# microsoft/ORBIT-Dataset

Measured on AMD Instinct MI355X. Metric: query frames/sec per task (224×224, 5-way ProtoNet) + frame accuracy vs ref, higher is better.
Workload: dtype f32

## Files before the change

include/orbit_hip.h:

```cpp
#ifndef ORBIT_HIP_H
#define ORBIT_HIP_H

#include <stddef.h>
#include <stdint.h>

#ifdef __cplusplus
extern "C" {
#endif

typedef struct orbit_extractor orbit_extractor_t;
typedef struct orbit_filmgen orbit_filmgen_t;
typedef void* orbit_stream_t;

#define ORBIT_OK 0
#define ORBIT_ERR_ARG (-1)
#define ORBIT_ERR_HIP (-2)
#define ORBIT_ERR_STATE (-3)
#define ORBIT_ERR_NOMEM (-4)

#define ORBIT_ACT_NONE 0
#define ORBIT_ACT_RELU 1
#define ORBIT_ACT_SILU 2
#define ORBIT_ACT_ELU 3

// ... 37 lines not shown

int orbit_extractor_load(orbit_extractor_t* fe, const char* key, const float* data, size_t numel);
int orbit_extractor_load_async(orbit_extractor_t* fe, const char* key, const float* device_data, size_t numel,
                               orbit_stream_t stream);
int orbit_extractor_load_all_async(orbit_extractor_t* fe, const float* const* device_ptrs, int n, orbit_stream_t stream);
int orbit_extractor_finalize(orbit_extractor_t* fe, orbit_stream_t stream);

int orbit_extractor_output_size(const orbit_extractor_t* fe);
int orbit_extractor_film_slots(const orbit_extractor_t* fe);
int orbit_extractor_film_slot_channels(const orbit_extractor_t* fe, int slot);
const char* orbit_extractor_film_slot_name(const orbit_extractor_t* fe, int slot);
int orbit_extractor_film_size(const orbit_extractor_t* fe);

size_t orbit_extractor_workspace_bytes(const orbit_extractor_t* fe, int B);
double orbit_extractor_macs_per_frame(const orbit_extractor_t* fe);

int orbit_extractor_forward(orbit_extractor_t* fe, const float* frames, int B,
                            const float* film_gamma, const float* film_beta,
                            float* feats, void* workspace, size_t workspace_bytes, orbit_stream_t stream);

int orbit_filmgen_create(int n_gen, int z_dim, int hidden, const int* out_size, const int* kind,
                         const int* dst_offset, orbit_filmgen_t** out);
void orbit_filmgen_destroy(orbit_filmgen_t* g);
int orbit_filmgen_load(orbit_filmgen_t* g, int gen, const char* tensor, const float* data, size_t numel);
int orbit_filmgen_load_all_async(orbit_filmgen_t* g, const float* const* device_ptrs, int n, orbit_stream_t stream);
int orbit_filmgen_forward(orbit_filmgen_t* g, const float* z, float* film_gamma, float* film_beta,
                          float* l2, orbit_stream_t stream);

int orbit_op_conv2d(const float* x, int x_nchw, const float* w, float* y,
                    const float* scale, const float* shift, const float* residual, const float* gate,
                    int B, int H, int W, int Cin, int Cout, int KH, int KW, int stride,
                    int pad_top, int pad_left, int Ho, int Wo, int act, int pool2,
                    orbit_stream_t stream);
int orbit_op_dwconv2d(const float* x, const float* w, float* y, const float* scale, const float* shift,
                      int B, int H, int W, int C, int K, int stride, int pad_top, int pad_left,
                      int Ho, int Wo, int act, orbit_stream_t stream);
int orbit_op_conv2d_train(const float* x, int x_nchw, const float* w, float* y, const float* gate, int B, int H, int W,
                          int Cin, int Cout, int KH, int KW, int stride, int pad_top, int pad_left, int Ho, int Wo,
                          float* stats, int* stat_blocks, orbit_stream_t stream);
int orbit_op_dwconv2d_train(const float* x, const float* w, float* y, const float* in_scale, const float* in_shift,
                            int in_act, int B, int H, int W, int C, int K, int stride, int pad_top, int pad_left, int Ho,
                            int Wo, float* stats, orbit_stream_t stream);
int orbit_op_maxpool2d(const float* x, float* y, int B, int H, int W, int C, int K, int stride, int pad,
                       int Ho, int Wo, orbit_stream_t stream);
int orbit_op_avgpool(const float* x, float* y, int B, int HW, int C, orbit_stream_t stream);
int orbit_op_se_gate(const float* pooled, const float* w1, const float* b1, const float* w2,
                     const float* b2, float* gate, int B, int C, int R, orbit_stream_t stream);

int orbit_op_mbconv_front_partials(int H, int W, int Cin, int mid, int K, int stride);
int orbit_op_mbconv_front(const float* x, const float* w1, const float* scale1, const float* shift1,
                          const float* wdw, const float* scale2, const float* shift2, float* y, float* pool_partial,
                          int B, int H, int W, int Cin, int mid, int K, int stride, int pad_top, int pad_left,
                          int Ho, int Wo, orbit_stream_t stream);
int orbit_op_stem_dw_front_partials(int H, int W, int mid);
int orbit_op_stem_dw_front(const float* frames, const float* w_stem, const float* scale1, const float* shift1,
                           const float* wdw, const float* scale2, const float* shift2, float* y, float* pool_partial,
                           int B, int FH, int FW, int spad_top, int spad_left, int H, int W, int mid, int pad_top,
                           int pad_left, int Ho, int Wo, orbit_stream_t stream);

int orbit_dense_rows(const float* x, int R, int in, const float* W, const float* b, int out, int act,
                     const float* residual, float* y, orbit_stream_t stream);
int orbit_spd_inverse(const float* A, float* Ainv, int n, int batch, orbit_stream_t stream);
size_t orbit_mahalanobis_workspace_bytes(int N, int M, int D, int C);
int orbit_mahalanobis_configure(const float* features, const int64_t* labels, const int64_t* class_ids, int N, int D,
                                int C, float* means, float* task_mean, float* precisions, float* task_precision,
                                void* workspace, size_t workspace_bytes, orbit_stream_t stream);
// ... 115 lines not shown
```

orbit-dataset_amd/_lib.py:

```python
import ctypes
import os
from ctypes import c_char_p, c_double, c_float, c_int, c_size_t, c_void_p, POINTER

_HERE = os.path.dirname(os.path.abspath(__file__))
LIB_PATH = os.path.join(_HERE, "lib", "liborbit_hip.so")

_lib = None

P = c_void_p
_SIGNATURES = {
    "orbit_version": (c_int, []),
    "orbit_last_error": (c_char_p, []),
    "orbit_device_count": (c_int, []),
    "orbit_set_option": (c_int, [c_char_p, c_int]),
    "orbit_get_option": (c_int, [c_char_p]),
    "orbit_label_set": (c_int, [P, c_int, P, c_int, P, P]),
    "orbit_proto_configure": (c_int, [P, P, P, c_int, c_int, c_int, c_int, c_int, P, P, P]),
    "orbit_proto_finalize": (c_int, [P, P, c_int, c_int, c_int, c_int, P, P, P]),
    "orbit_proto_predict": (c_int, [P, P, P, c_int, c_int, c_int, c_int, c_int, c_float, c_int, P, P, P]),
    "orbit_mean_pool": (c_int, [P, c_int, c_int, c_int, P, P]),
    "orbit_set_mean": (c_int, [P, c_int, c_int, P, P]),
    "orbit_history_mean_pool": (c_int, [P, c_int, c_int, c_int, P, P]),
    "orbit_extractor_create": (c_int, [c_char_p, c_int, c_int, POINTER(c_void_p)]),
    "orbit_extractor_create_ex": (c_int, [c_char_p, c_int, c_int, c_int, POINTER(c_void_p)]),
    "orbit_extractor_destroy": (None, [P]),
    "orbit_extractor_num_params": (c_int, [P]),
    "orbit_extractor_param_name": (c_char_p, [P, c_int]),
    "orbit_extractor_param_numel": (c_size_t, [P, c_int]),
    "orbit_extractor_load": (c_int, [P, c_char_p, P, c_size_t]),
    "orbit_extractor_load_async": (c_int, [P, c_char_p, P, c_size_t, P]),
    "orbit_extractor_load_all_async": (c_int, [P, P, c_int, P]),
    "orbit_extractor_finalize": (c_int, [P, P]),
    "orbit_extractor_output_size": (c_int, [P]),
    "orbit_extractor_film_slots": (c_int, [P]),
    "orbit_extractor_film_slot_channels": (c_int, [P, c_int]),
    "orbit_extractor_film_slot_name": (c_char_p, [P, c_int]),
    "orbit_extractor_film_size": (c_int, [P]),
    "orbit_extractor_workspace_bytes": (c_size_t, [P, c_int]),
    "orbit_extractor_macs_per_frame": (c_double, [P]),
    "orbit_extractor_forward": (c_int, [P, P, c_int, P, P, P, P, c_size_t, P]),
    "orbit_filmgen_create": (c_int, [c_int, c_int, c_int, POINTER(c_int), POINTER(c_int), POINTER(c_int),
                                     POINTER(c_void_p)]),
    "orbit_filmgen_destroy": (None, [P]),
    "orbit_filmgen_load": (c_int, [P, c_int, c_char_p, P, c_size_t]),
    "orbit_filmgen_load_all_async": (c_int, [P, P, c_int, P]),
    "orbit_filmgen_forward": (c_int, [P, P, P, P, P, P]),
    "orbit_op_conv2d": (c_int, [P, c_int, P, P, P, P, P, P] + [c_int] * 14 + [P]),
    "orbit_op_dwconv2d": (c_int, [P, P, P, P, P] + [c_int] * 11 + [P]),
    "orbit_op_conv2d_train": (c_int, [P, c_int, P, P, P] + [c_int] * 12 + [P, POINTER(c_int), P]),
    "orbit_op_dwconv2d_train": (c_int, [P, P, P, P, P] + [c_int] * 11 + [P, P]),
    "orbit_op_maxpool2d": (c_int, [P, P] + [c_int] * 9 + [P]),
    "orbit_op_avgpool": (c_int, [P, P, c_int, c_int, c_int, P]),
    "orbit_op_se_gate": (c_int, [P, P, P, P, P, P, c_int, c_int, c_int, P]),
    "orbit_op_mbconv_front": (c_int, [P] * 9 + [c_int] * 11 + [P]),
    "orbit_op_mbconv_front_partials": (c_int, [c_int] * 6),
    "orbit_op_stem_dw_front_partials": (c_int, [c_int] * 3),
    "orbit_op_stem_dw_front": (c_int, [P] * 9 + [c_int] * 12 + [P]),
    "orbit_dense_rows": (c_int, [P, c_int, c_int, P, P, c_int, c_int, P, P, P]),
    "orbit_spd_inverse": (c_int, [P, P, c_int, c_int, P]),
    "orbit_mahalanobis_workspace_bytes": (c_size_t, [c_int, c_int, c_int, c_int]),
    "orbit_mahalanobis_configure": (c_int, [P, P, P, c_int, c_int, c_int, P, P, P, P, P, c_size_t, P]),
    "orbit_mahalanobis_predict": (c_int, [P, P, P, c_int, c_int, c_int, c_float, P, P, c_size_t, P]),
    "orbit_mahalanobis_predict_backward": (c_int, [P, P, P, P, c_int, c_int, c_int, c_float, P, P, c_size_t, P]),
    "orbit_extractor_supports_training": (c_int, [P]),
    "orbit_extractor_tape_bytes": (c_size_t, [P, c_int]),
    "orbit_extractor_backward_workspace_bytes": (c_size_t, [P, c_int]),
    "orbit_extractor_grad_floats": (c_size_t, [P]),
    "orbit_extractor_param_offset": (c_size_t, [P, c_int]),
    "orbit_extractor_bn_stat_floats": (c_size_t, [P]),
    "orbit_extractor_export_bn_stats": (c_int, [P, P, P]),
    "orbit_extractor_train_forward": (c_int, [P, P, c_int, P, P, c_int, c_float, P, P, c_size_t, P]),
    "orbit_extractor_train_forward_ex": (c_int, [P, P, c_int, P, P, c_int, c_float, P, P, c_size_t, c_int, P]),
    "orbit_extractor_apply_deferred_bn_stats": (c_int, [P, P, c_size_t, c_int, c_float, P]),
    "orbit_extractor_backward": (c_int, [P, P, c_int, P, P, c_int, P, P, c_size_t, P, c_int, P, P, P, c_size_t, P]),
    "orbit_filmgen_grad_floats": (c_size_t, [P]),
    "orbit_filmgen_param_offset": (c_size_t, [P, c_int, c_char_p]),
    "orbit_filmgen_backward": (c_int, [P, P, P, P, P, P, P, P]),
    "orbit_proto_predict_backward": (c_int, [P, P, P, c_int, c_int, c_int, c_int, c_float, c_int, P, P]),
    "orbit_linear_head_backward": (c_int, [P, P, c_int, c_int, c_int, c_float, P, P, P]),
    "orbit_cross_entropy_forward": (c_int, [P, P, c_int, c_int, c_int, P, P, P, P]),
    "orbit_cross_entropy_backward": (c_int, [P, P, P, c_int, c_int, c_int, P, P]),
# ... 160 lines not shown
```

orbit-dataset_amd/build.py:

```python
import hashlib
import os
import subprocess
import sys
from concurrent.futures import ThreadPoolExecutor

HERE = os.path.dirname(os.path.abspath(__file__))
CSRC = os.path.join(HERE, "csrc")
LIBDIR = os.path.join(HERE, "lib")
OBJDIR = os.path.join(HERE, "build")
LIB = os.path.join(LIBDIR, "liborbit_hip.so")
INCLUDE = os.path.join(os.path.dirname(HERE), "include")

SOURCES = ["head.hip", "heads_extra.hip", "loss.hip", "conv_igemm.hip", "pw_rgemm.hip", "conv_bf3.hip", "ops.hip", "film.hip", "ingest.hip", "mbconv_rows.hip", "stem.hip", "extractor.hip", "train_ops.hip", "train_mbconv.hip", "conv_wgrad.hip", "extractor_train.hip",
           "comm.hip"]
HIPCC = os.environ.get("HIPCC", "/opt/rocm/bin/hipcc")
FLAGS = ["--offload-arch=gfx950", "-O3", "-std=c++17", "-fPIC", "-Wall", "-Wno-unused-function",
         "-I", INCLUDE, "-I", "/opt/rocm/include"]


def _runtime_libdir():
    if os.environ.get("ORBIT_SYSTEM_ROCM") == "1":
        return "/opt/rocm/lib"
    try:
        import torch
        d = os.path.join(os.path.dirname(torch.__file__), "lib")
        if os.path.exists(os.path.join(d, "libamdhip64.so")):
            return d
    except Exception:
        pass
    return "/opt/rocm/lib"


RTLIB = _runtime_libdir()
LINK = ["-shared", "-fPIC", "--offload-arch=gfx950", "-no-hip-rt", "-L" + RTLIB, "-lamdhip64", "-lrccl",
        "-Wl,-rpath," + RTLIB, "-Wl,--no-undefined"]


def _digest(paths):
    root = os.path.dirname(HERE)
    h = hashlib.sha256()
    for p in sorted(paths):
        with open(p, "rb") as f:
            h.update(os.path.relpath(p, root).encode())
            h.update(f.read())
    h.update(" ".join(x.replace(root, "<repo>") for x in FLAGS + LINK).encode())
    return h.hexdigest()
# ... 48 lines not shown
```

orbit-dataset_amd/csrc/common.h:

```cpp
#pragma once
#include <hip/hip_runtime.h>
#include <cstdarg>
#include <cstdio>
#include <cstdint>
#include <cstring>
#include "../../include/orbit_hip.h"

namespace orbit {

char* err_buf();
int set_err(int code, const char* fmt, ...);
int get_option(const char* name);
int option_epoch();

#define ORBIT_HIP_CHECK(expr)                                                                  \
    do {                                                                                       \
        hipError_t _e = (expr);                                                                \
        if (_e != hipSuccess)                                                                  \
            return ::orbit::set_err(ORBIT_ERR_HIP, "%s failed: %s (%s:%d)", #expr,             \
                                    hipGetErrorString(_e), __FILE__, __LINE__);                \
    } while (0)

#define ORBIT_LAUNCH_CHECK()                                                                   \
    do {                                                                                       \
// ... 36 lines not shown
    const float* gate;
    int B, H, W, Cin, Cout, KH, KW, stride, pad_t, pad_l, Ho, Wo;
    int act;
    int pool2;
    int x_nchw;
    float prof_flop_scale = 1.f;
    float* splitk_ws = nullptr;
    float* stats = nullptr;
    int* stats_blocks = nullptr;
    bool stats_only = false;
    float* y_raw = nullptr;
};
inline size_t conv_stats_floats(size_t M, int Cout) { return ((M + 31) / 32) * 2 * (size_t)Cout; }
int conv_splitk(const ConvDesc& d);
size_t conv_splitk_floats(const ConvDesc& d);

struct ConvPackGeom {
    int cin_pad;
    int kt;
    int cout_pad;
};
ConvPackGeom conv_pack_geom(int Cin, int Cout, int KH, int KW, int x_nchw);
size_t conv_packed_floats(int Cin, int Cout, int KH, int KW, int x_nchw);
int conv_pack_weights(const float* w_oihw, float* w_packed, int Cin, int Cout, int KH, int KW,
                      int x_nchw, hipStream_t s);
int launch_conv(const ConvDesc& d, hipStream_t s);
size_t conv_frag_floats(int Cin, int Cout, int KH, int KW, int x_nchw);
int conv_frag_pack_weights(const float* w_oihw, float* w_frag, int Cin, int Cout, hipStream_t s);
bool pw_rgemm_supported(const ConvDesc& d);
bool conv_bf3_supported(const ConvDesc& d);
int launch_conv_bf3(const ConvDesc& d, hipStream_t s);
bool pw_rgemm_preferred(const ConvDesc& d);
int launch_pw_rgemm(const ConvDesc& d, hipStream_t s);
bool conv_prof_enabled();
int prof_start(const char* name, double flops, double bytes, hipStream_t s, double silu = 0.0);
void prof_stop(int idx, hipStream_t s);

struct DwBnBwd {
    const float* y = nullptr;
    const float* mean = nullptr;
    const float* invstd = nullptr;
    const float* scale = nullptr;
    const float* shift = nullptr;
    int act = 0;
    float* partial = nullptr;
    int* nblk = nullptr;
    float* wgrad_partial = nullptr;
    int* wgrad_rows = nullptr;
};
int dwconv_se_chunks(int Ho);
int launch_dwconv_se(const float* x, const float* w_khwc, float* y, const float* scale, const float* shift,
                     float* pool_partial, int B, int H, int W, int C, int K, int stride, int pad_t, int pad_l, int Ho,
                     int Wo, int act, hipStream_t s, int stats = 0, const float* in_scale = nullptr,
                     const float* in_shift = nullptr, int in_act = 0, const DwBnBwd* bnb = nullptr);
int launch_se_gate2(const float* partial, int chunks, int HW, const float* w1, const float* b1, const float* w2t,
                    const float* b2, float* gate, int B, int C, int R, hipStream_t s, float* pooled_out = nullptr);
int launch_transpose(const float* in, float* out, int rows, int cols, hipStream_t s);
bool stem_direct_supported(int Cin, int Cout, int K, int stride, int W, int act);
int launch_stem_direct(const float* frames, const float* w_oihw, const float* scale, const float* shift, float* y, int B,
                       int H, int W, int pad_t, int pad_l, int Ho, int Wo, hipStream_t s);
bool mbconv_rows_supported(int H, int W, int Cin, int mid, int K, int stride);
int mbconv_rows_tiles(int H, int W, int Cin, int mid, int K, int stride);
int launch_mbconv_rows(const float* x, const float* w1, const float* sc1, const float* sh1, const float* wdw,
                       const float* sc2, const float* sh2, float* y, float* pool, int B, int H, int W, int Cin, int mid,
                       int K, int stride, int pad_t, int pad_l, int Ho, int Wo, hipStream_t s, int plan_tiles = 0,
                       bool raw_stats = false);
// ... 114 lines not shown
```

orbit-dataset_amd/csrc/extractor.hip:

```cpp
#include <chrono>
#include <cstdlib>

#include "extractor.h"

using namespace orbit;

static int conv_out(int H, int K, int stride, int pad) { return (H + 2 * pad - K) / stride + 1; }
static void same_pad(int H, int K, int stride, int& Ho, int& pad_before) {
    Ho = (H + stride - 1) / stride;
    const int total = std::max((Ho - 1) * stride + K - H, 0);
    pad_before = total / 2;
}

static int build_resnet18(orbit_extractor* fe, int H, int W) {
    fe->out_size = 512;
    int h = conv_out(H, 7, 2, 3), w = conv_out(W, 7, 2, 3);
    int bn = fe->add_bn("bn1", 64, 1e-5f, true);
    fe->add_conv("conv1.weight", bn, -1, 0, -1, H, W, 3, 64, 7, 2, 3, 3, h, w, ORBIT_ACT_RELU, 0, 1, 0);
    {
        Op o;
        o.kind = OP_MAXPOOL, o.in = 0, o.out = 1, o.H = h, o.W = w, o.Cin = 64, o.Cout = 64;
        o.pool_k = 3, o.stride = 2, o.pool_pad = 1;
        o.Ho = conv_out(h, 3, 2, 1), o.Wo = conv_out(w, 3, 2, 1);
        h = o.Ho, w = o.Wo;
// ... 472 lines not shown
    }
    hit->stamp = ++fe->graph_clock;
    if (hit->exec == nullptr) {
        hipGraph_t graph = nullptr;
        if (fe->cap_stream == nullptr)
            ORBIT_HIP_CHECK(hipStreamCreateWithFlags(&fe->cap_stream, hipStreamNonBlocking));
        if (hipStreamBeginCapture(fe->cap_stream, hipStreamCaptureModeThreadLocal) != hipSuccess) {
            (void)hipGetLastError();
            return run_plan(fe, frames, B, film_gamma, film_beta, feats, workspace, s);
        }
        const int rc = run_plan(fe, frames, B, film_gamma, film_beta, feats, workspace, fe->cap_stream);
        const hipError_t ce = hipStreamEndCapture(fe->cap_stream, &graph);
        if (rc != ORBIT_OK) {
            if (graph) (void)hipGraphDestroy(graph);
            return rc;
        }
        if (ce != hipSuccess || graph == nullptr) {
            (void)hipGetLastError();
            return run_plan(fe, frames, B, film_gamma, film_beta, feats, workspace, s);
        }
        hipGraphExec_t exec = nullptr;
        const hipError_t ie = hipGraphInstantiate(&exec, graph, nullptr, nullptr, 0);
        (void)hipGraphDestroy(graph);
        if (ie != hipSuccess || exec == nullptr) {
            (void)hipGetLastError();
            return run_plan(fe, frames, B, film_gamma, film_beta, feats, workspace, s);
        }
        hit->exec = exec;
    }
    ORBIT_HIP_CHECK(hipGraphLaunch(hit->exec, s));
    return ORBIT_OK;
}

static int run_plan(orbit_extractor_t* fe, const float* frames, int B, const float* film_gamma, const float* film_beta,
                    float* feats, void* workspace, hipStream_t s) {
    const WsLayout L = ws_layout(fe, B);
    char* ws = static_cast<char*>(workspace);
    auto buf = [&](int id) -> float* {
        if (id == -1) return const_cast<float*>(frames);
        if (id == 100) return feats;
        if (id == 101) return reinterpret_cast<float*>(ws + L.pooled);
        if (id == 102) return reinterpret_cast<float*>(ws + L.gate);
        return reinterpret_cast<float*>(ws + L.buf[id]);
    };
    const float* scale = fe->d_fold;
    const float* shift = fe->d_fold + fe->fold_floats;
    if (film_gamma && fe->film_size > 0) {
        float* fs = reinterpret_cast<float*>(ws + L.fold);
        dim3 grid((unsigned)fe->bns.size(), 2);
        const int rec = prof_start("bn_fold_film", 0.0, 4.0 * 6.0 * fe->fold_floats, s);
        bn_fold_all_kernel<<<grid, 256, 0, s>>>(fe->d_bn, fe->d_pool, film_gamma, film_beta, fs, fs + fe->fold_floats);
        prof_stop(rec, s);
        ORBIT_LAUNCH_CHECK();
        scale = fs, shift = fs + fe->fold_floats;
    }
    for (size_t oi = 0; oi < fe->ops.size(); ++oi) {
        const Op& o = fe->ops[oi];
        int rc = ORBIT_OK;
        switch (o.kind) {
            case OP_CONV: {
                if (o.x_nchw && !o.pool2 && o.res < 0 && o.bn >= 0 &&
                    stem_direct_supported(o.Cin, o.Cout, o.KH, o.stride, o.W, o.act) && o.KH == o.KW) {
                    rc = launch_stem_direct(buf(o.in), fe->d_pool + fe->params[o.weight].off, scale + fe->bns[o.bn].fold_off,
                                            shift + fe->bns[o.bn].fold_off, buf(o.out), B, o.H, o.W, o.pad_t, o.pad_l, o.Ho,
                                            o.Wo, s);
                    break;
                }
                ConvDesc d;
                d.x = buf(o.in), d.w_packed = fe->d_packed + o.packed_off, d.y = buf(o.out);
                d.w_frag = o.frag_off != SIZE_MAX ? fe->d_packed + o.frag_off : nullptr;
                d.scale = o.bn >= 0 ? scale + fe->bns[o.bn].fold_off : nullptr;
                d.shift = o.bn >= 0 ? shift + fe->bns[o.bn].fold_off : nullptr;
                d.residual = o.res >= 0 ? buf(o.res) : nullptr;
                d.gate = o.use_gate ? buf(102) : nullptr;
                d.B = B, d.H = o.H, d.W = o.W, d.Cin = o.Cin, d.Cout = o.Cout, d.KH = o.KH, d.KW = o.KW;
                d.stride = o.stride, d.pad_t = o.pad_t, d.pad_l = o.pad_l, d.Ho = o.Ho, d.Wo = o.Wo;
                d.act = o.act, d.pool2 = o.pool2, d.x_nchw = o.x_nchw;
                d.splitk_ws = reinterpret_cast<float*>(ws + L.splitk);
                rc = launch_conv(d, s);
                break;
            }
            case OP_DWCONV:
                rc = launch_dwconv_se(buf(o.in), fe->d_packed + o.packed_off, buf(o.out),
                                      scale + fe->bns[o.bn].fold_off, shift + fe->bns[o.bn].fold_off,
                                      o.pool_partial ? buf(101) : nullptr, B, o.H, o.W, o.Cin, o.KH, o.stride, o.pad_t,
                                      o.pad_l, o.Ho, o.Wo, o.act, s);
                break;
            case OP_MBFRONT:
                if (o.stem)
                    rc = launch_stem_rows(buf(o.in), fe->d_packed + o.packed_off2, scale + fe->bns[o.bn].fold_off,
                                          shift + fe->bns[o.bn].fold_off, fe->d_packed + o.packed_off,
                                          scale + fe->bns[o.bn2].fold_off, shift + fe->bns[o.bn2].fold_off, buf(o.out),
                                          buf(101), B, o.stem_h, o.stem_w, o.stem_pt, o.stem_pl, o.H, o.W, s, o.se_chunks);
                else
                    rc = launch_mbconv_rows(buf(o.in), fe->d_pool + fe->params[o.weight].off,
                                            scale + fe->bns[o.bn].fold_off, shift + fe->bns[o.bn].fold_off,
                                            fe->d_packed + o.packed_off, scale + fe->bns[o.bn2].fold_off,
                                            shift + fe->bns[o.bn2].fold_off, buf(o.out), buf(101), B, o.H, o.W, o.Cin,
                                            o.Cout, o.KH, o.stride, o.pad_t, o.pad_l, o.Ho, o.Wo, s, o.se_chunks);
                break;
            case OP_MAXPOOL:
                rc = launch_maxpool(buf(o.in), buf(o.out), B, o.H, o.W, o.Cin, o.pool_k, o.stride, o.pool_pad, o.Ho,
                                    o.Wo, s);
                break;
            case OP_AVGPOOL:
                rc = launch_avgpool(buf(o.in), buf(o.out), B, o.H * o.W, o.Cin, s);
                break;
            case OP_SE:
                rc = launch_se_gate2(buf(101), o.se_chunks, o.se_hw, fe->d_pool + fe->params[o.se_w1].off,
                                     fe->d_pool + fe->params[o.se_b1].off, fe->d_packed + o.packed_off,
                                     fe->d_pool + fe->params[o.se_b2].off, buf(102), B, o.Cin, o.R, s);
                break;
        }
        if (rc != ORBIT_OK) return rc;
    }
    return ORBIT_OK;
}

}
```

orbit-dataset_amd/csrc/ops.hip:

```cpp
#include "common.h"
#include <algorithm>

namespace orbit {

using v4f = __attribute__((ext_vector_type(4))) float;

__device__ __forceinline__ float act_fn(float v, int act) {
    if (act == ORBIT_ACT_RELU) return fmaxf(v, 0.f);
    if (act == ORBIT_ACT_SILU) return v * __builtin_amdgcn_rcpf(1.0f + __expf(-v));
    return v;
}

struct DwInXf {
    const float* scale;
    const float* shift;
    int act;
};
struct DwBnbVec {
    v4f sc, sh, mu, is;
};
__device__ __forceinline__ v4f dw_bnb(v4f dx, v4f yv, const DwBnbVec& b, int act, v4f& s0, v4f& s1) {
    const v4f z = yv * b.sc + b.sh;
    v4f g = dx;
    if (act == ORBIT_ACT_SILU) {
#pragma unroll
        for (int k = 0; k < 4; ++k) {
            const float sg = __builtin_amdgcn_rcpf(1.0f + __expf(-z[k]));
            g[k] *= sg * (1.0f + z[k] * (1.0f - sg));
        }
    } else if (act == ORBIT_ACT_RELU) {
#pragma unroll
        for (int k = 0; k < 4; ++k) g[k] = z[k] > 0.f ? g[k] : 0.f;
    }
// ... 526 lines not shown
                const int wo = g * 4 + j;
                if (wo < Wo) {
                    if (BNB) {
                        *reinterpret_cast<v4f*>(yb + ((size_t)ho * Wo + wo) * C) = dw_bnb(acc[j], yv[j], bv, bnb.act, psum, psq);
                    } else {
                        v4f o = acc[j] * sc + sh;
                        o[0] = act_fn(o[0], act), o[1] = act_fn(o[1], act), o[2] = act_fn(o[2], act), o[3] = act_fn(o[3], act);
                        *reinterpret_cast<v4f*>(yb + ((size_t)ho * Wo + wo) * C) = o;
                        psum += o;
                        if (STATS) psq += o * o;
                    }
                }
            }
        }
    }
    if (pool_partial == nullptr) return;
    red[p * cs4 + lc] = psum;
    __syncthreads();
    const size_t prow = ((size_t)b * gridDim.y + chunk) * (STATS ? 2 : 1);
    if (tid < cs4) {
        v4f t = red[tid];
        for (int l = 1; l < P; ++l) t += red[l * cs4 + tid];
        *reinterpret_cast<v4f*>(pool_partial + prow * C + c0 + tid * 4) = t;
    }
    if (STATS) {
        __syncthreads();
        red[p * cs4 + lc] = psq;
        __syncthreads();
        if (tid < cs4) {
            v4f t = red[tid];
            for (int l = 1; l < P; ++l) t += red[l * cs4 + tid];
            *reinterpret_cast<v4f*>(pool_partial + (prow + 1) * C + c0 + tid * 4) = t;
        }
    }
}

template <int CTRL, int ROW_MASK>
__device__ __forceinline__ float se_dpp_add(float v) {
    return v + __int_as_float(__builtin_amdgcn_update_dpp(0, __float_as_int(v), CTRL, ROW_MASK, 0xf, false));
}
__device__ __forceinline__ float se_wave_sum(float v) {
    v = se_dpp_add<0xB1, 0xf>(v);
    v = se_dpp_add<0x4E, 0xf>(v);
    v = se_dpp_add<0x141, 0xf>(v);
    v = se_dpp_add<0x140, 0xf>(v);
    v = se_dpp_add<0x142, 0xa>(v);
    v = se_dpp_add<0x143, 0xc>(v);
    return __int_as_float(__builtin_amdgcn_readlane(__float_as_int(v), 63));
}

template <int NT, int U>
__device__ __forceinline__ void se_gate_frame(const float* __restrict__ partial, int chunks, float inv_hw,
                                              const float* __restrict__ w1, const float* __restrict__ b1,
                                              const float* __restrict__ w2t, const float* __restrict__ b2,
                                              float* __restrict__ gate, int C, int R, float* __restrict__ pooled_out, float* sm2) {
    v4f* sp4 = reinterpret_cast<v4f*>(sm2);
    float* hid = sm2 + C;
    const int tid = threadIdx.x;
    const int C4 = C >> 2;
    const v4f* part4 = reinterpret_cast<const v4f*>(partial);
    const int parts = C4 <= NT / 2 ? NT / C4 : 1;
    if (parts > 1 && chunks > 8) {
        v4f* tmp = reinterpret_cast<v4f*>(sm2 + ((C + R + 3) & ~3));
        const int q = tid % C4, part = tid / C4;
        if (part < parts) {
            v4f s = {0.f, 0.f, 0.f, 0.f};
#pragma unroll 4
            for (int k = part; k < chunks; k += parts) s += part4[(size_t)k * C4 + q];
            tmp[part * C4 + q] = s;
        }
        __syncthreads();
        if (tid < C4) {
            v4f s = tmp[tid];
            for (int g = 1; g < parts; ++g) s += tmp[g * C4 + tid];
            sp4[tid] = s * inv_hw;
        }
    } else {
        for (int c4 = tid; c4 < C4; c4 += NT) {
            v4f s = {0.f, 0.f, 0.f, 0.f};
#pragma unroll 8
            for (int k = 0; k < chunks; ++k) s += part4[(size_t)k * C4 + c4];
            sp4[c4] = s * inv_hw;
        }
    }
    __syncthreads();
    if (pooled_out != nullptr)
        for (int c4 = tid; c4 < C4; c4 += NT) reinterpret_cast<v4f*>(pooled_out)[c4] = sp4[c4];
    const int lane = tid & 63, wave = tid >> 6;
    const v4f* w14 = reinterpret_cast<const v4f*>(w1);
    for (int r0 = wave; r0 < R; r0 += U * (NT / 64)) {
        float acc[U];
#pragma unroll
        for (int u = 0; u < U; ++u) acc[u] = 0.f;
        for (int cb = 0; cb < C4; cb += 320) {
            v4f wv[U][5], pv[5];
#pragma unroll
            for (int j = 0; j < 5; ++j) {
                const int c4 = cb + lane + 64 * j;
                const bool ok = c4 < C4;
                pv[j] = ok ? sp4[c4] : (v4f){0.f, 0.f, 0.f, 0.f};
#pragma unroll
                for (int u = 0; u < U; ++u) {
                    const int r = r0 + (NT / 64) * u;
                    wv[u][j] = (ok && r < R) ? w14[(size_t)r * C4 + c4] : (v4f){0.f, 0.f, 0.f, 0.f};
                }
            }
#pragma unroll
            for (int u = 0; u < U; ++u)
#pragma unroll
                for (int j = 0; j < 5; ++j) {
                    const v4f t = wv[u][j] * pv[j];
                    acc[u] += (t[0] + t[1]) + (t[2] + t[3]);
                }
        }
#pragma unroll
        for (int u = 0; u < U; ++u) {
            const int r = r0 + (NT / 64) * u;
            const float sum = se_wave_sum(acc[u]);
            if (r < R && lane == 0) {
                const float t = sum + b1[r];
                hid[r] = t / (1.0f + expf(-t));
            }
        }
    }
    __syncthreads();
    const v4f* w24 = reinterpret_cast<const v4f*>(w2t);
    for (int c4 = tid; c4 < C4; c4 += NT) {
        v4f a = *reinterpret_cast<const v4f*>(b2 + 4 * c4);
        int r = 0;
        for (; r + 8 <= R; r += 8) {
            v4f wv[8];
#pragma unroll
            for (int u = 0; u < 8; ++u) wv[u] = w24[(size_t)(r + u) * C4 + c4];
#pragma unroll
            for (int u = 0; u < 8; ++u) a += wv[u] * hid[r + u];
        }
        for (; r < R; ++r) a += w24[(size_t)r * C4 + c4] * hid[r];
        v4f g;
#pragma unroll
        for (int q = 0; q < 4; ++q) g[q] = 1.0f / (1.0f + expf(-a[q]));
        reinterpret_cast<v4f*>(gate)[c4] = g;
    }
}

template <int NT>
__global__ __launch_bounds__(NT) void se_gate2_kernel(const float* __restrict__ partial, int chunks, float inv_hw,
                                                       const float* __restrict__ w1, const float* __restrict__ b1,
                                                       const float* __restrict__ w2t, const float* __restrict__ b2,
                                                       float* __restrict__ gate, int C, int R,
                                                       float* __restrict__ pooled_out) {
    extern __shared__ __attribute__((aligned(16))) float sm2[];
    const int b = blockIdx.x;
    se_gate_frame<NT, 4>(partial + (size_t)b * chunks * C, chunks, inv_hw, w1, b1, w2t, b2, gate + (size_t)b * C, C, R,
                         pooled_out ? pooled_out + (size_t)b * C : nullptr, sm2);
}

__global__ __launch_bounds__(256) void transpose_kernel(const float* __restrict__ in, float* __restrict__ out, int rows,
                                                        int cols) {
    const int total = rows * cols;
    for (int i = blockIdx.x * 256 + threadIdx.x; i < total; i += gridDim.x * 256) {
        const int r = i / cols, c = i % cols;
        out[(size_t)c * rows + r] = in[i];
    }
}

__global__ __launch_bounds__(256) void maxpool_kernel(const float* __restrict__ x, float* __restrict__ y,
                                                      int B, int H, int W, int C, int K, int stride, int pad,
                                                      int Ho, int Wo) {
    const int C4 = C >> 2;
    const size_t total = (size_t)B * Ho * Wo * C4;
    for (size_t i = (size_t)blockIdx.x * 256 + threadIdx.x; i < total; i += (size_t)gridDim.x * 256) {
        const unsigned iu = (unsigned)i, r1 = iu / (unsigned)C4, r2 = r1 / (unsigned)Wo, bu = r2 / (unsigned)Ho;
        const int c = (int)(iu - r1 * C4) * 4, wo = (int)(r1 - r2 * Wo), ho = (int)(r2 - bu * Ho), b = (int)bu;
        const float* xb = x + (size_t)b * H * W * C + c;
// ... 378 lines not shown
```

Measured before the change: 36890.

## Fuse SE gate computation into following pointwise projection conv kernel

```diff
diff --git a/include/orbit_hip.h b/include/orbit_hip.h
--- a/include/orbit_hip.h
+++ b/include/orbit_hip.h
@@ -93,6 +93,10 @@
                     int B, int H, int W, int Cin, int Cout, int KH, int KW, int stride,
                     int pad_top, int pad_left, int Ho, int Wo, int act, int pool2,
                     orbit_stream_t stream);
+int orbit_op_pw_stream(const float* x, const float* w, const float* scale, const float* shift, const float* residual,
+                       const float* partial, int chunks, const float* w1, const float* b1, const float* w2t, const float* b2,
+                       int R, float* y, float* gate_out, int B, int H, int W, int Cin, int Cout, orbit_stream_t stream);
+int orbit_pw_stream_supported(int Cin, int Cout, int H, int W);
 int orbit_op_dwconv2d(const float* x, const float* w, float* y, const float* scale, const float* shift,
                       int B, int H, int W, int C, int K, int stride, int pad_top, int pad_left,
                       int Ho, int Wo, int act, orbit_stream_t stream);
diff --git a/orbit-dataset_amd/_lib.py b/orbit-dataset_amd/_lib.py
--- a/orbit-dataset_amd/_lib.py
+++ b/orbit-dataset_amd/_lib.py
@@ -47,6 +47,8 @@
     "orbit_filmgen_forward": (c_int, [P, P, P, P, P, P]),
     "orbit_op_conv2d": (c_int, [P, c_int, P, P, P, P, P, P] + [c_int] * 14 + [P]),
     "orbit_op_dwconv2d": (c_int, [P, P, P, P, P] + [c_int] * 11 + [P]),
+    "orbit_op_pw_stream": (c_int, [P] * 6 + [c_int] + [P] * 4 + [c_int, P, P] + [c_int] * 5 + [P]),
+    "orbit_pw_stream_supported": (c_int, [c_int] * 4),
     "orbit_op_conv2d_train": (c_int, [P, c_int, P, P, P] + [c_int] * 12 + [P, POINTER(c_int), P]),
     "orbit_op_dwconv2d_train": (c_int, [P, P, P, P, P] + [c_int] * 11 + [P, P]),
     "orbit_op_maxpool2d": (c_int, [P, P] + [c_int] * 9 + [P]),
diff --git a/orbit-dataset_amd/build.py b/orbit-dataset_amd/build.py
--- a/orbit-dataset_amd/build.py
+++ b/orbit-dataset_amd/build.py
@@ -11,7 +11,7 @@
 LIB = os.path.join(LIBDIR, "liborbit_hip.so")
 INCLUDE = os.path.join(os.path.dirname(HERE), "include")
 
-SOURCES = ["head.hip", "heads_extra.hip", "loss.hip", "conv_igemm.hip", "pw_rgemm.hip", "conv_bf3.hip", "ops.hip", "film.hip", "ingest.hip", "mbconv_rows.hip", "stem.hip", "extractor.hip", "train_ops.hip", "train_mbconv.hip", "conv_wgrad.hip", "extractor_train.hip",
+SOURCES = ["head.hip", "heads_extra.hip", "loss.hip", "conv_igemm.hip", "pw_rgemm.hip", "pw_stream.hip", "conv_bf3.hip", "ops.hip", "film.hip", "ingest.hip", "mbconv_rows.hip", "stem.hip", "extractor.hip", "train_ops.hip", "train_mbconv.hip", "conv_wgrad.hip", "extractor_train.hip",
            "comm.hip"]
 HIPCC = os.environ.get("HIPCC", "/opt/rocm/bin/hipcc")
 FLAGS = ["--offload-arch=gfx950", "-O3", "-std=c++17", "-fPIC", "-Wall", "-Wno-unused-function",
diff --git a/orbit-dataset_amd/csrc/common.h b/orbit-dataset_amd/csrc/common.h
--- a/orbit-dataset_amd/csrc/common.h
+++ b/orbit-dataset_amd/csrc/common.h
@@ -92,6 +92,22 @@
 int launch_conv_bf3(const ConvDesc& d, hipStream_t s);
 bool pw_rgemm_preferred(const ConvDesc& d);
 int launch_pw_rgemm(const ConvDesc& d, hipStream_t s);
+struct PwStreamDesc {
+    const float* x;
+    const float* w_packed;
+    float* y;
+    const float* scale;
+    const float* shift;
+    const float* residual = nullptr;
+    const float* partial;
+    int chunks, se_hw;
+    const float *w1, *b1, *w2t, *b2;
+    int R;
+    float* gate_out = nullptr;
+    int B, H, W, Cin, Cout;
+};
+bool pw_stream_supported(int Cin, int Cout, int H, int W);
+int launch_pw_stream(const PwStreamDesc& d, hipStream_t s);
 bool conv_prof_enabled();
 int prof_start(const char* name, double flops, double bytes, hipStream_t s, double silu = 0.0);
 void prof_stop(int idx, hipStream_t s);
diff --git a/orbit-dataset_amd/csrc/extractor.hip b/orbit-dataset_amd/csrc/extractor.hip
--- a/orbit-dataset_amd/csrc/extractor.hip
+++ b/orbit-dataset_amd/csrc/extractor.hip
@@ -528,6 +528,14 @@
     return ORBIT_OK;
 }
 
+static bool se_in_projection(const orbit_extractor_t* fe, size_t i) {
+    if (!get_option("conv_rgemm") || i + 1 >= fe->ops.size() || fe->ops[i].kind != OP_SE) return false;
+    const Op& c = fe->ops[i + 1];
+    return c.kind == OP_CONV && c.use_gate && c.Cin == fe->ops[i].Cin && c.KH == 1 && c.KW == 1 && c.stride == 1 &&
+           c.pad_t == 0 && c.pad_l == 0 && !c.x_nchw && !c.pool2 && c.act == ORBIT_ACT_NONE && c.bn >= 0 &&
+           c.Ho == c.H && c.Wo == c.W && pw_stream_supported(c.Cin, c.Cout, c.H, c.W);
+}
+
 static int run_plan(orbit_extractor_t* fe, const float* frames, int B, const float* film_gamma, const float* film_beta,
                     float* feats, void* workspace, hipStream_t s) {
     const WsLayout L = ws_layout(fe, B);
@@ -560,6 +568,19 @@
                     rc = launch_stem_direct(buf(o.in), fe->d_pool + fe->params[o.weight].off, scale + fe->bns[o.bn].fold_off,
                                             shift + fe->bns[o.bn].fold_off, buf(o.out), B, o.H, o.W, o.pad_t, o.pad_l, o.Ho,
                                             o.Wo, s);
+                    break;
+                }
+                if (oi > 0 && se_in_projection(fe, oi - 1)) {
+                    const Op& se = fe->ops[oi - 1];
+                    PwStreamDesc d;
+                    d.x = buf(o.in), d.w_packed = fe->d_packed + o.packed_off, d.y = buf(o.out);
+                    d.scale = scale + fe->bns[o.bn].fold_off, d.shift = shift + fe->bns[o.bn].fold_off;
+                    d.residual = o.res >= 0 ? buf(o.res) : nullptr;
+                    d.partial = buf(101), d.chunks = se.se_chunks, d.se_hw = se.se_hw;
+                    d.w1 = fe->d_pool + fe->params[se.se_w1].off, d.b1 = fe->d_pool + fe->params[se.se_b1].off;
+                    d.w2t = fe->d_packed + se.packed_off, d.b2 = fe->d_pool + fe->params[se.se_b2].off, d.R = se.R;
+                    d.B = B, d.H = o.H, d.W = o.W, d.Cin = o.Cin, d.Cout = o.Cout;
+                    rc = launch_pw_stream(d, s);
                     break;
                 }
                 ConvDesc d;
@@ -603,6 +624,7 @@
                 rc = launch_avgpool(buf(o.in), buf(o.out), B, o.H * o.W, o.Cin, s);
                 break;
             case OP_SE:
+                if (se_in_projection(fe, oi)) break;
                 rc = launch_se_gate2(buf(101), o.se_chunks, o.se_hw, fe->d_pool + fe->params[o.se_w1].off,
                                      fe->d_pool + fe->params[o.se_b1].off, fe->d_packed + o.packed_off,
                                      fe->d_pool + fe->params[o.se_b2].off, buf(102), B, o.Cin, o.R, s);
diff --git a/orbit-dataset_amd/csrc/ops.hip b/orbit-dataset_amd/csrc/ops.hip
--- a/orbit-dataset_amd/csrc/ops.hip
+++ b/orbit-dataset_amd/csrc/ops.hip
@@ -1,4 +1,5 @@
 #include "common.h"
+#include "se_gate.h"
 #include <algorithm>
 
 namespace orbit {
@@ -591,114 +592,6 @@
             for (int l = 1; l < P; ++l) t += red[l * cs4 + tid];
             *reinterpret_cast<v4f*>(pool_partial + (prow + 1) * C + c0 + tid * 4) = t;
         }
-    }
-}
-
-template <int CTRL, int ROW_MASK>
-__device__ __forceinline__ float se_dpp_add(float v) {
-    return v + __int_as_float(__builtin_amdgcn_update_dpp(0, __float_as_int(v), CTRL, ROW_MASK, 0xf, false));
-}
-__device__ __forceinline__ float se_wave_sum(float v) {
-    v = se_dpp_add<0xB1, 0xf>(v);
-    v = se_dpp_add<0x4E, 0xf>(v);
-    v = se_dpp_add<0x141, 0xf>(v);
-    v = se_dpp_add<0x140, 0xf>(v);
-    v = se_dpp_add<0x142, 0xa>(v);
-    v = se_dpp_add<0x143, 0xc>(v);
-    return __int_as_float(__builtin_amdgcn_readlane(__float_as_int(v), 63));
-}
-
-template <int NT, int U>
-__device__ __forceinline__ void se_gate_frame(const float* __restrict__ partial, int chunks, float inv_hw,
-                                              const float* __restrict__ w1, const float* __restrict__ b1,
-                                              const float* __restrict__ w2t, const float* __restrict__ b2,
-                                              float* __restrict__ gate, int C, int R, float* __restrict__ pooled_out, float* sm2) {
-    v4f* sp4 = reinterpret_cast<v4f*>(sm2);
-    float* hid = sm2 + C;
-    const int tid = threadIdx.x;
-    const int C4 = C >> 2;
-    const v4f* part4 = reinterpret_cast<const v4f*>(partial);
-    const int parts = C4 <= NT / 2 ? NT / C4 : 1;
-    if (parts > 1 && chunks > 8) {
-        v4f* tmp = reinterpret_cast<v4f*>(sm2 + ((C + R + 3) & ~3));
-        const int q = tid % C4, part = tid / C4;
-        if (part < parts) {
-            v4f s = {0.f, 0.f, 0.f, 0.f};
-#pragma unroll 4
-            for (int k = part; k < chunks; k += parts) s += part4[(size_t)k * C4 + q];
-            tmp[part * C4 + q] = s;
-        }
-        __syncthreads();
-        if (tid < C4) {
-            v4f s = tmp[tid];
-            for (int g = 1; g < parts; ++g) s += tmp[g * C4 + tid];
-            sp4[tid] = s * inv_hw;
-        }
-    } else {
-        for (int c4 = tid; c4 < C4; c4 += NT) {
-            v4f s = {0.f, 0.f, 0.f, 0.f};
-#pragma unroll 8
-            for (int k = 0; k < chunks; ++k) s += part4[(size_t)k * C4 + c4];
-            sp4[c4] = s * inv_hw;
-        }
-    }
-    __syncthreads();
-    if (pooled_out != nullptr)
-        for (int c4 = tid; c4 < C4; c4 += NT) reinterpret_cast<v4f*>(pooled_out)[c4] = sp4[c4];
-    const int lane = tid & 63, wave = tid >> 6;
-    const v4f* w14 = reinterpret_cast<const v4f*>(w1);
-    for (int r0 = wave; r0 < R; r0 += U * (NT / 64)) {
-        float acc[U];
-#pragma unroll
-        for (int u = 0; u < U; ++u) acc[u] = 0.f;
-        for (int cb = 0; cb < C4; cb += 320) {
-            v4f wv[U][5], pv[5];
-#pragma unroll
-            for (int j = 0; j < 5; ++j) {
-                const int c4 = cb + lane + 64 * j;
-                const bool ok = c4 < C4;
-                pv[j] = ok ? sp4[c4] : (v4f){0.f, 0.f, 0.f, 0.f};
-#pragma unroll
-                for (int u = 0; u < U; ++u) {
-                    const int r = r0 + (NT / 64) * u;
-                    wv[u][j] = (ok && r < R) ? w14[(size_t)r * C4 + c4] : (v4f){0.f, 0.f, 0.f, 0.f};
-                }
-            }
-#pragma unroll
-            for (int u = 0; u < U; ++u)
-#pragma unroll
-                for (int j = 0; j < 5; ++j) {
-                    const v4f t = wv[u][j] * pv[j];
-                    acc[u] += (t[0] + t[1]) + (t[2] + t[3]);
-                }
-        }
-#pragma unroll
-        for (int u = 0; u < U; ++u) {
-            const int r = r0 + (NT / 64) * u;
-            const float sum = se_wave_sum(acc[u]);
-            if (r < R && lane == 0) {
-                const float t = sum + b1[r];
-                hid[r] = t / (1.0f + expf(-t));
-            }
-        }
-    }
-    __syncthreads();
-    const v4f* w24 = reinterpret_cast<const v4f*>(w2t);
-    for (int c4 = tid; c4 < C4; c4 += NT) {
-        v4f a = *reinterpret_cast<const v4f*>(b2 + 4 * c4);
-        int r = 0;
-        for (; r + 8 <= R; r += 8) {
-            v4f wv[8];
-#pragma unroll
-            for (int u = 0; u < 8; ++u) wv[u] = w24[(size_t)(r + u) * C4 + c4];
-#pragma unroll
-            for (int u = 0; u < 8; ++u) a += wv[u] * hid[r + u];
-        }
-        for (; r < R; ++r) a += w24[(size_t)r * C4 + c4] * hid[r];
-        v4f g;
-#pragma unroll
-        for (int q = 0; q < 4; ++q) g[q] = 1.0f / (1.0f + expf(-a[q]));
-        reinterpret_cast<v4f*>(gate)[c4] = g;
     }
 }
 
diff --git a/orbit-dataset_amd/csrc/pw_stream.hip b/orbit-dataset_amd/csrc/pw_stream.hip
--- /dev/null
+++ b/orbit-dataset_amd/csrc/pw_stream.hip
@@ -0,0 +1,227 @@
+#include <algorithm>
+#include <type_traits>
+#include "common.h"
+#include "se_gate.h"
+
+namespace orbit {
+
+using f32x4 = __attribute__((ext_vector_type(4))) float;
+
+struct PwsParams {
+    const float* x;
+    const float* w;
+    float* y;
+    const float* scale;
+    const float* shift;
+    const float* residual;
+    const float* partial;
+    const float *w1, *b1, *w2t, *b2;
+    float* gate_out;
+    float inv_hw;
+    int KT, chunks, R, HW, Cout;
+    int tiles;
+    int bpf;
+};
+
+template <int KC, int NG, int TP>
+__global__ __launch_bounds__(256) void pw_stream_kernel(PwsParams p) {
+    constexpr int K = 16 * KC;
+    extern __shared__ __attribute__((aligned(16))) float sm[];
+    f32x4* wl = reinterpret_cast<f32x4*>(sm);
+    float* gl = sm + KC * NG * 256;
+    float* sg = gl + K;
+    const int tid = threadIdx.x, lane = tid & 63, wave = tid >> 6;
+    const int q = lane >> 4;
+    const int b = blockIdx.x / p.bpf, seg = blockIdx.x - b * p.bpf;
+    const int t_beg = (int)((long)seg * p.tiles / p.bpf), t_end = (int)((long)(seg + 1) * p.tiles / p.bpf);
+    const size_t pix0 = (size_t)b * p.HW + (lane & 15);
+    const bool has_res = p.residual != nullptr;
+
+    auto has = [&](int s) { return t_beg + (4 * s + wave) * TP < t_end; };
+    auto tile_of = [&](int s, int u) { return t_beg + (4 * s + wave) * TP + u; };
+    auto row_of = [&](int s, int u) {
+        const int t = tile_of(s, u);
+        return pix0 + (size_t)16 * (t < t_end ? t : tile_of(s, 0));
+    };
+
+    f32x4 xa[TP][KC];
+    if (has(0)) {
+#pragma unroll
+        for (int u = 0; u < TP; ++u) {
+            const float* px = p.x + row_of(0, u) * K + 4 * q;
+#pragma unroll
+            for (int c = 0; c < KC; ++c) xa[u][c] = *reinterpret_cast<const f32x4*>(px + 16 * c);
+        }
+    }
+
+    for (int i = tid; i < KC * NG * 64; i += 256) {
+        const int l = i & 63, g = (i >> 6) % NG, c = (i >> 6) / NG;
+        wl[i] = *reinterpret_cast<const f32x4*>(p.w + (size_t)(16 * g + (l & 15)) * p.KT + 16 * c + 4 * (l >> 4));
+    }
+    se_gate_frame<256, 4>(p.partial + (size_t)b * p.chunks * K, p.chunks, p.inv_hw, p.w1, p.b1, p.w2t, p.b2, gl, K, p.R,
+                          nullptr, sg);
+    __syncthreads();
+    if (p.gate_out != nullptr && seg == 0)
+        for (int c4 = tid; c4 < K / 4; c4 += 256)
+            reinterpret_cast<f32x4*>(p.gate_out + (size_t)b * K)[c4] = reinterpret_cast<const f32x4*>(gl)[c4];
+
+    f32x4 sc[NG], sh[NG];
+#pragma unroll
+    for (int g = 0; g < NG; ++g) {
+        const int ch = 16 * g + 4 * q;
+        const bool ok = ch < p.Cout;
+        sc[g] = ok ? *reinterpret_cast<const f32x4*>(p.scale + ch) : (f32x4){0.f, 0.f, 0.f, 0.f};
+        sh[g] = ok ? *reinterpret_cast<const f32x4*>(p.shift + ch) : (f32x4){0.f, 0.f, 0.f, 0.f};
+    }
+
+    auto step = [&](int s, auto refill) {
+        constexpr bool REFILL = decltype(refill)::value;
+        __asm__ volatile("" ::: "memory");
+        size_t row[TP], nrow[TP];
+#pragma unroll
+        for (int u = 0; u < TP; ++u) row[u] = row_of(s, u), nrow[u] = REFILL ? row_of(s + 1, u) : row[u];
+        f32x4 rr[TP][NG];
+        if (has_res)
+#pragma unroll
+            for (int u = 0; u < TP; ++u)
+#pragma unroll
+                for (int g = 0; g < NG; ++g) {
+                    const int ch = 16 * g + 4 * q;
+                    rr[u][g] = *reinterpret_cast<const f32x4*>(p.residual + row[u] * p.Cout + (ch < p.Cout ? ch : 0));
+                }
+        f32x4 acc[TP][NG];
+#pragma unroll
+        for (int u = 0; u < TP; ++u)
+#pragma unroll
+            for (int g = 0; g < NG; ++g) acc[u][g] = (f32x4){0.f, 0.f, 0.f, 0.f};
+#pragma unroll
+        for (int c = 0; c < KC; ++c) {
+            const f32x4 gv = *reinterpret_cast<const f32x4*>(gl + 16 * c + 4 * q);
+            f32x4 xv[TP];
+#pragma unroll
+            for (int u = 0; u < TP; ++u) {
+                xv[u] = xa[u][c] * gv;
+                if (REFILL) xa[u][c] = *reinterpret_cast<const f32x4*>(p.x + nrow[u] * K + 4 * q + 16 * c);
+            }
+#pragma unroll
+            for (int g = 0; g < NG; ++g) {
+                const f32x4 wv = wl[(c * NG + g) * 64 + lane];
+#pragma unroll
+                for (int e = 0; e < 4; ++e)
+#pragma unroll
+                    for (int u = 0; u < TP; ++u)
+                        acc[u][g] = __builtin_amdgcn_mfma_f32_16x16x4f32(wv[e], xv[u][e], acc[u][g], 0, 0, 0);
+            }
+        }
+#pragma unroll
+        for (int u = 0; u < TP; ++u) {
+            if (tile_of(s, u) >= t_end) continue;
+#pragma unroll
+            for (int g = 0; g < NG; ++g) {
+                const int ch = 16 * g + 4 * q;
+                if (ch >= p.Cout) continue;
+                f32x4 o = acc[u][g] * sc[g] + sh[g];
+                if (has_res) o += rr[u][g];
+                *reinterpret_cast<f32x4*>(p.y + row[u] * p.Cout + ch) = o;
+            }
+        }
+    };
+    int s = 0;
+    for (; has(s + 1); ++s) step(s, std::true_type{});
+    if (has(s)) step(s, std::false_type{});
+}
+
+namespace {
+struct PwsVariant {
+    int kc, ng, tp;
+    void (*fn)(PwsParams);
+};
+const PwsVariant kVariants[] = {
+    {2, 1, 2, pw_stream_kernel<2, 1, 2>},
+    {6, 2, 1, pw_stream_kernel<6, 2, 1>},
+    {9, 2, 1, pw_stream_kernel<9, 2, 1>},
+    {9, 3, 1, pw_stream_kernel<9, 3, 1>},
+};
+const PwsVariant* find_variant(int Cin, int Cout) {
+    if (Cin % 16 != 0 || Cout % 8 != 0 || Cout > 48) return nullptr;
+    for (const PwsVariant& v : kVariants)
+        if (v.kc == Cin / 16 && v.ng == cdiv(Cout, 16)) return &v;
+    return nullptr;
+}
+}
+
+bool pw_stream_supported(int Cin, int Cout, int H, int W) {
+    return find_variant(Cin, Cout) != nullptr && (H * W) % 16 == 0;
+}
+
+int launch_pw_stream(const PwStreamDesc& d, hipStream_t s) {
+    ORBIT_REQUIRE(d.x && d.w_packed && d.y && d.scale && d.shift && d.partial && d.w1 && d.b1 && d.w2t && d.b2,
+                  "pw_stream: null pointer");
+    ORBIT_REQUIRE(pw_stream_supported(d.Cin, d.Cout, d.H, d.W), "pw_stream: unsupported layer %d -> %d @%dx%d", d.Cin, d.Cout,
+                  d.H, d.W);
+    ORBIT_REQUIRE(d.B > 0 && d.chunks > 0 && d.se_hw > 0 && d.R > 0, "pw_stream: bad sizes");
+    const PwsVariant& v = *find_variant(d.Cin, d.Cout);
+    const ConvPackGeom geom = conv_pack_geom(d.Cin, d.Cout, 1, 1, 0);
+    ORBIT_REQUIRE(geom.kt >= d.Cin && geom.cout_pad >= 16 * v.ng, "pw_stream: packed filter too small");
+    PwsParams p;
+    p.x = d.x, p.w = d.w_packed, p.y = d.y, p.scale = d.scale, p.shift = d.shift, p.residual = d.residual;
+    p.partial = d.partial, p.w1 = d.w1, p.b1 = d.b1, p.w2t = d.w2t, p.b2 = d.b2, p.gate_out = d.gate_out;
+    p.inv_hw = 1.0f / (float)d.se_hw;
+    p.KT = geom.kt, p.chunks = d.chunks, p.R = d.R, p.HW = d.H * d.W, p.Cout = d.Cout;
+    p.tiles = p.HW / 16;
+    p.bpf = std::max(1, std::min(p.tiles, cdiv(p.tiles, 24 * v.tp)));
+    ORBIT_REQUIRE((long long)d.B * p.bpf < (1ll << 31), "pw_stream: grid too large");
+    const size_t lds = ((size_t)v.kc * v.ng * 256 + d.Cin + ((d.Cin + d.R + 3) & ~3) + 4 * 256) * sizeof(float);
+    const double M = (double)d.B * p.HW;
+    char name[48];
+    snprintf(name, sizeof(name), "conv_pw_stream<%dx%d%s>", d.Cin, d.Cout, d.residual ? ",res" : "");
+    const int rec = prof_start(name, 2.0 * M * d.Cin * d.Cout,
+                               4.0 * (M * d.Cin + M * d.Cout * (d.residual ? 2.0 : 1.0) + (double)d.B * d.chunks * d.Cin), s);
+    hipLaunchKernelGGL(v.fn, dim3((unsigned)(d.B * p.bpf)), dim3(256), lds, s, p);
+    prof_stop(rec, s);
+    ORBIT_LAUNCH_CHECK();
+    return ORBIT_OK;
+}
+
+}
+
+extern "C" {
+
+int orbit_pw_stream_supported(int Cin, int Cout, int H, int W) { return orbit::pw_stream_supported(Cin, Cout, H, W) ? 1 : 0; }
+
+int orbit_op_pw_stream(const float* x, const float* w, const float* scale, const float* shift, const float* residual,
+                       const float* partial, int chunks, const float* w1, const float* b1, const float* w2t, const float* b2,
+                       int R, float* y, float* gate_out, int B, int H, int W, int Cin, int Cout, orbit_stream_t stream) {
+    using namespace orbit;
+    ORBIT_REQUIRE(x && w && scale && shift && partial && w1 && b1 && w2t && b2 && y, "op_pw_stream: null pointer");
+    hipStream_t s = (hipStream_t)stream;
+    const bool fused = get_option("conv_rgemm") && pw_stream_supported(Cin, Cout, H, W);
+    const size_t nfl = (conv_packed_floats(Cin, Cout, 1, 1, 0) + 63) & ~(size_t)63;
+    const size_t ffl = conv_frag_floats(Cin, Cout, 1, 1, 0);
+    const size_t gfl = (fused || gate_out) ? 0 : (size_t)B * Cin;
+    float* wp = nullptr;
+    ORBIT_HIP_CHECK(hipMallocAsync(reinterpret_cast<void**>(&wp), (nfl + ffl + gfl) * sizeof(float), s));
+    int rc = conv_pack_weights(w, wp, Cin, Cout, 1, 1, 0, s);
+    if (rc == ORBIT_OK && ffl) rc = conv_frag_pack_weights(w, wp + nfl, Cin, Cout, s);
+    if (rc == ORBIT_OK && fused) {
+        PwStreamDesc d;
+        d.x = x, d.w_packed = wp, d.y = y, d.scale = scale, d.shift = shift, d.residual = residual;
+        d.partial = partial, d.chunks = chunks, d.se_hw = H * W, d.w1 = w1, d.b1 = b1, d.w2t = w2t, d.b2 = b2, d.R = R;
+        d.gate_out = gate_out, d.B = B, d.H = H, d.W = W, d.Cin = Cin, d.Cout = Cout;
+        rc = launch_pw_stream(d, s);
+    } else if (rc == ORBIT_OK) {
+        float* gate = gate_out ? gate_out : wp + nfl + ffl;
+        rc = launch_se_gate2(partial, chunks, H * W, w1, b1, w2t, b2, gate, B, Cin, R, s);
+        if (rc == ORBIT_OK) {
+            ConvDesc d;
+            d.x = x, d.w_packed = wp, d.w_frag = ffl ? wp + nfl : nullptr, d.y = y, d.scale = scale, d.shift = shift;
+            d.residual = residual, d.gate = gate, d.B = B, d.H = H, d.W = W, d.Cin = Cin, d.Cout = Cout, d.KH = d.KW = 1;
+            d.stride = 1, d.pad_t = d.pad_l = 0, d.Ho = H, d.Wo = W, d.act = ORBIT_ACT_NONE, d.pool2 = 0, d.x_nchw = 0;
+            rc = launch_conv(d, s);
+        }
+    }
+    (void)hipFreeAsync(wp, s);
+    return rc;
+}
+
+}
diff --git a/orbit-dataset_amd/csrc/se_gate.h b/orbit-dataset_amd/csrc/se_gate.h
--- /dev/null
+++ b/orbit-dataset_amd/csrc/se_gate.h
@@ -0,0 +1,116 @@
+#pragma once
+#include "common.h"
+
+namespace orbit {
+
+using v4f = __attribute__((ext_vector_type(4))) float;
+
+template <int CTRL, int ROW_MASK>
+__device__ __forceinline__ float se_dpp_add(float v) {
+    return v + __int_as_float(__builtin_amdgcn_update_dpp(0, __float_as_int(v), CTRL, ROW_MASK, 0xf, false));
+}
+__device__ __forceinline__ float se_wave_sum(float v) {
+    v = se_dpp_add<0xB1, 0xf>(v);
+    v = se_dpp_add<0x4E, 0xf>(v);
+    v = se_dpp_add<0x141, 0xf>(v);
+    v = se_dpp_add<0x140, 0xf>(v);
+    v = se_dpp_add<0x142, 0xa>(v);
+    v = se_dpp_add<0x143, 0xc>(v);
+    return __int_as_float(__builtin_amdgcn_readlane(__float_as_int(v), 63));
+}
+
+template <int NT, int U>
+__device__ __forceinline__ void se_gate_frame(const float* __restrict__ partial, int chunks, float inv_hw,
+                                              const float* __restrict__ w1, const float* __restrict__ b1,
+                                              const float* __restrict__ w2t, const float* __restrict__ b2,
+                                              float* __restrict__ gate, int C, int R, float* __restrict__ pooled_out, float* sm2) {
+    v4f* sp4 = reinterpret_cast<v4f*>(sm2);
+    float* hid = sm2 + C;
+    const int tid = threadIdx.x;
+    const int C4 = C >> 2;
+    const v4f* part4 = reinterpret_cast<const v4f*>(partial);
+    const int parts = C4 <= NT / 2 ? NT / C4 : 1;
+    if (parts > 1 && chunks > 8) {
+        v4f* tmp = reinterpret_cast<v4f*>(sm2 + ((C + R + 3) & ~3));
+        const int q = tid % C4, part = tid / C4;
+        if (part < parts) {
+            v4f s = {0.f, 0.f, 0.f, 0.f};
+#pragma unroll 4
+            for (int k = part; k < chunks; k += parts) s += part4[(size_t)k * C4 + q];
+            tmp[part * C4 + q] = s;
+        }
+        __syncthreads();
+        if (tid < C4) {
+            v4f s = tmp[tid];
+            for (int g = 1; g < parts; ++g) s += tmp[g * C4 + tid];
+            sp4[tid] = s * inv_hw;
+        }
+    } else {
+        for (int c4 = tid; c4 < C4; c4 += NT) {
+            v4f s = {0.f, 0.f, 0.f, 0.f};
+#pragma unroll 8
+            for (int k = 0; k < chunks; ++k) s += part4[(size_t)k * C4 + c4];
+            sp4[c4] = s * inv_hw;
+        }
+    }
+    __syncthreads();
+    if (pooled_out != nullptr)
+        for (int c4 = tid; c4 < C4; c4 += NT) reinterpret_cast<v4f*>(pooled_out)[c4] = sp4[c4];
+    const int lane = tid & 63, wave = tid >> 6;
+    const v4f* w14 = reinterpret_cast<const v4f*>(w1);
+    for (int r0 = wave; r0 < R; r0 += U * (NT / 64)) {
+        float acc[U];
+#pragma unroll
+        for (int u = 0; u < U; ++u) acc[u] = 0.f;
+        for (int cb = 0; cb < C4; cb += 320) {
+            v4f wv[U][5], pv[5];
+#pragma unroll
+            for (int j = 0; j < 5; ++j) {
+                const int c4 = cb + lane + 64 * j;
+                const bool ok = c4 < C4;
+                pv[j] = ok ? sp4[c4] : (v4f){0.f, 0.f, 0.f, 0.f};
+#pragma unroll
+                for (int u = 0; u < U; ++u) {
+                    const int r = r0 + (NT / 64) * u;
+                    wv[u][j] = (ok && r < R) ? w14[(size_t)r * C4 + c4] : (v4f){0.f, 0.f, 0.f, 0.f};
+                }
+            }
+#pragma unroll
+            for (int u = 0; u < U; ++u)
+#pragma unroll
+                for (int j = 0; j < 5; ++j) {
+                    const v4f t = wv[u][j] * pv[j];
+                    acc[u] += (t[0] + t[1]) + (t[2] + t[3]);
+                }
+        }
+#pragma unroll
+        for (int u = 0; u < U; ++u) {
+            const int r = r0 + (NT / 64) * u;
+            const float sum = se_wave_sum(acc[u]);
+            if (r < R && lane == 0) {
+                const float t = sum + b1[r];
+                hid[r] = t / (1.0f + expf(-t));
+            }
+        }
+    }
+    __syncthreads();
+    const v4f* w24 = reinterpret_cast<const v4f*>(w2t);
+    for (int c4 = tid; c4 < C4; c4 += NT) {
+        v4f a = *reinterpret_cast<const v4f*>(b2 + 4 * c4);
+        int r = 0;
+        for (; r + 8 <= R; r += 8) {
+            v4f wv[8];
+#pragma unroll
+            for (int u = 0; u < 8; ++u) wv[u] = w24[(size_t)(r + u) * C4 + c4];
+#pragma unroll
+            for (int u = 0; u < 8; ++u) a += wv[u] * hid[r + u];
+        }
+        for (; r < R; ++r) a += w24[(size_t)r * C4 + c4] * hid[r];
+        v4f g;
+#pragma unroll
+        for (int q = 0; q < 4; ++q) g[q] = 1.0f / (1.0f + expf(-a[q]));
+        reinterpret_cast<v4f*>(gate)[c4] = g;
+    }
+}
+
+}
```

New measurement: 37800 (median of 6 runs). +2.5%, better.
